# y00njaekim/CMU-11785-IDL-1.58bit-ASR

Hardware: AMD Instinct MI355X
Metric: mel-frames/sec (Conformer-S 1.58-bit train step) (higher is better)
Workload: dtype fp32; 1 GPU; conformer-s-1.58bit-train-step; global_batch=32, execution=hip-graph, per_gpu_batch=32, frames=1000, d_model=144, blocks=16, d_ff=576, heads=4, vocab=5004, parallelism=dp1, passes=teacher 2-bit + student 1-bit + SP, conv_pointwise=fp32 (reference)

## Files before the change

cmu-11785-idl-1.58bit-asr_amd/csrc/capi.hip:

```cpp
#include <float.h>

#include <algorithm>
#include <vector>

#include "../../include/onebit_hip.h"
#include "ob_launch.h"
#include <stdint.h>

using namespace ob;

namespace {

constexpr int kAbiVersion = 4;

inline hipStream_t as_stream(void* s) { return reinterpret_cast<hipStream_t>(s); }

inline bool aligned4(const void* p) { return (reinterpret_cast<uintptr_t>(p) & 3) == 0; }
inline bool misaligned8(const void* p) { return (reinterpret_cast<uintptr_t>(p) & 7) != 0; }

inline int check_bits(int bits) { return (bits == 1 || bits == 2) ? OB_OK : OB_ERR_BITWIDTH; }

inline int launched() {
  const hipError_t e = hipGetLastError();
  return e == hipSuccess ? OB_OK : OB_ERR_HIP;
// ... 2059 lines not shown
  if ((dgamma || dbeta) && ws_bytes < layernorm_bwd_workspace(rows, d)) return OB_ERR_WORKSPACE;
  if (!aligned4(dy) || !aligned4(x) || !aligned4(dx) || !aligned4(dres) || !aligned4(dy2) ||
      !aligned4(lens))
    return OB_ERR_ALIGN;
  if (dy2) {
    if (!(p_drop >= 0.0f && p_drop < 1.0f)) return OB_ERR_SHAPE;
    if (lens && (T < 1 || T > 0x7fffffff || rows % T)) return OB_ERR_SHAPE;
    if (p_drop > 0.0f && !rng) return OB_ERR_NULL;
  }
  LnGradScale gs{dy2, rscale, p_drop, rng, (uint64_t)rng_offset,
                 reinterpret_cast<const int*>(lens), (int)T};
  const LnDefer df{static_cast<LnParamEntry*>(table), (int)slot};
  launch_layernorm_bwd(dy, x, gamma, mean, rstd, rows, d, dres, dx, dgamma, dbeta, ws,
                       as_stream(stream), &gs, &df);
  return launched();
}

namespace {
int relattn_check(int64_t Bt, int64_t P, int64_t T, int64_t H, int64_t d, float p_drop) {
  if (Bt < 1 || P < 1 || Bt % P != 0 || H < 1 || !relattn_supported(T, d)) return OB_ERR_SHAPE;
  if (Bt > 65535 || H > 65535 || !(p_drop >= 0.0f && p_drop < 1.0f)) return OB_ERR_SHAPE;
  return OB_OK;
}
}

int ob_relattn_fwd(const float* q, const float* k, const float* v, const float* pos,
                   const float* u, const float* vb, const int32_t* lens, int64_t Bt, int64_t P,
                   int64_t T, int64_t H, int64_t d, float p_drop, const int64_t* rng,
                   int64_t rng_offset, float* saved, float* probs, float* ctx, void* stream) {
  if (int st = relattn_check(Bt, P, T, H, d, p_drop)) return st;
  if (!q || !k || !v || !pos || !u || !vb || !lens || !ctx || (p_drop > 0.0f && !rng))
    return OB_ERR_NULL;
  if (((uintptr_t)saved & 15) || ((uintptr_t)probs & 15)) return OB_ERR_ALIGN;
  launch_relattn_fwd(q, k, v, pos, u, vb, lens, Bt, P, T, H, d, p_drop,
                     reinterpret_cast<const uint64_t*>(rng), (uint64_t)rng_offset, saved, probs,
                     ctx, as_stream(stream));
  return launched();
}

int64_t ob_relattn_saved_elems(int64_t Bt, int64_t T, int64_t H, int64_t d) {
  if (Bt < 1 || H < 1 || !relattn_supported(T, d)) return 0;
  return relattn_saved_elems(Bt, T, H, d);
}

size_t ob_relattn_bwd_workspace(int64_t Bt, int64_t T, int64_t H, int64_t d) {
  if (Bt < 1 || H < 1 || !relattn_supported(T, d)) return 0;
  return align_up(relattn_bwd_workspace(Bt, T, H, d));
}

int ob_relattn_set_bwd_mode(int mode) { return relattn_set_flash(mode); }

int ob_tgemm_set_colloop(int on) { return tgemm_set_colloop(on); }

int64_t ob_relattn_probs_elems(int64_t Bt, int64_t T, int64_t H) {
  if (Bt < 1 || H < 1 || T < 1) return 0;
  return relattn_probs_elems(Bt, T, H);
}

int ob_relattn_bwd(const float* dctx, const float* ctx, const float* q, const float* k,
                   const float* v, const float* pos, const float* u, const float* vb,
                   const int32_t* lens, int64_t Bt, int64_t P, int64_t T, int64_t H, int64_t d,
                   float p_drop, const int64_t* rng, int64_t rng_offset, const float* saved,
                   int64_t saved_elems, float* dq, float* dk, float* dv, float* dpos, float* du,
                   float* dvb, void* ws, size_t ws_bytes, void* stream) {
  if (int st = relattn_check(Bt, P, T, H, d, p_drop)) return st;
  if (!dctx || !ctx || !q || !k || !v || !pos || !u || !vb || !lens || !saved || !dq || !dk ||
      !dv || !dpos || !du || !dvb || !ws)
    return OB_ERR_NULL;
  if (saved_elems != relattn_saved_elems(Bt, T, H, d)) return OB_ERR_SHAPE;
  (void)rng;
  (void)rng_offset;
  if ((uintptr_t)saved & 15) return OB_ERR_ALIGN;
  if (ws_bytes < ob_relattn_bwd_workspace(Bt, T, H, d)) return OB_ERR_WORKSPACE;
  launch_relattn_bwd(dctx, ctx, q, k, v, pos, u, vb, lens, Bt, P, T, H, d, p_drop, saved, dq, dk,
                     dv, dpos, du, dvb, ws, as_stream(stream));
  return launched();
}

int ob_decattn_supported(int64_t Lq, int64_t Lk, int64_t dh) {
  return decattn_supported(Lq, Lk, dh) ? 1 : 0;
}

static int decattn_check(int64_t B, int64_t H, int64_t Lq, int64_t Lk, int64_t dh, int64_t sq,
                         int64_t sk, int64_t sv, float p_drop) {
  if (B < 0 || H < 1 || !decattn_supported(Lq, Lk, dh) || !(p_drop >= 0.0f && p_drop < 1.0f))
    return OB_ERR_SHAPE;
  if (sq < H * dh || sk < H * dh || sv < H * dh) return OB_ERR_SHAPE;
  if (B * H * Lq > INT32_MAX) return OB_ERR_SHAPE;
  return OB_OK;
}

int ob_decattn_fwd(const float* q, int64_t sq, const float* k, int64_t sk, const float* v,
                   int64_t sv, const uint8_t* kmask, int64_t causal, int64_t B, int64_t H,
                   int64_t Lq, int64_t Lk, int64_t dh, float p_drop, const int64_t* rng,
                   int64_t rng_offset, float* probs, float* ctx, void* stream) {
  if (int st = decattn_check(B, H, Lq, Lk, dh, sq, sk, sv, p_drop)) return st;
  if (B > 0 && (!q || !k || !v || !probs || !ctx || (p_drop > 0.0f && !rng))) return OB_ERR_NULL;
  if (!aligned4(q) || !aligned4(k) || !aligned4(v) || !aligned4(probs) ||
      (reinterpret_cast<uintptr_t>(ctx) & 15))
    return OB_ERR_ALIGN;
  launch_decattn_fwd(q, sq, k, sk, v, sv, kmask, causal ? 1 : 0, B, H, Lq, Lk, dh, p_drop,
                     reinterpret_cast<const uint64_t*>(rng), (uint64_t)rng_offset, probs, ctx,
                     as_stream(stream));
  return launched();
}

// ... 76 lines not shown
```

cmu-11785-idl-1.58bit-asr_amd/csrc/ob_launch.h:

```cpp
#pragma once

#include <hip/hip_runtime.h>
#include <stddef.h>
#include <stdint.h>

#include "../../include/onebit_hip.h"

namespace ob {

inline int64_t ceil_div(int64_t a, int64_t b) { return (a + b - 1) / b; }

void launch_quant_pack(const float* W, const float* alpha, int alpha_raw, int bits,
                       const int* bits_dev, int64_t N, int64_t K, uint32_t* codes,
                       uint32_t* codes_t, hipStream_t s);
int64_t quant_pack_item_blocks(int64_t N, int64_t K);
int64_t quant_pack_item_blocks16(int64_t N, int64_t K);
void launch_quant_pack_group(const ob_pack_item* items_dev, int n_items, int64_t total_blocks,
                             hipStream_t s);
void launch_quant_dequant(const float* W, const float* alpha, int alpha_raw, int bits, int64_t n,
                          float* W_hat, hipStream_t s);

int64_t ste_reduce_blocks(int64_t total);
void launch_ste_reduce(const float* part, int chunks, int64_t nk, const float* part_db,
                       int64_t n_db, const float* W, const float* alpha, int alpha_raw, int bits,
// ... 407 lines not shown
bool ctc_supported(int64_t S);
void launch_ctc_fwd(const float* lp, const int64_t* targets, const int64_t* in_len,
                    const int64_t* tg_len, int64_t B, int64_t T, int64_t V, int64_t S, int blank, int64_t G,
                    float* loss, float* ws, hipStream_t s);
void launch_ctc_bwd(const float* lp, const int64_t* targets, const int64_t* in_len,
                    const int64_t* tg_len, int64_t B, int64_t T, int64_t V, int64_t S, int blank, int64_t G,
                    const float* grad_out, float* grad, float* ws, hipStream_t s);
size_t ctc_logits_workspace_bytes(int64_t B, int64_t T, int64_t S);
void launch_ctc_logits_fwd(const float* x, const int64_t* targets, const int64_t* in_len,
                           const int64_t* tg_len, int64_t B, int64_t T, int64_t V, int64_t S,
                           int blank, int64_t G, float* loss, void* ws, hipStream_t s);
void launch_ctc_logits_bwd(const float* x, const int64_t* targets, const int64_t* in_len,
                           const int64_t* tg_len, int64_t B, int64_t T, int64_t V, int64_t S,
                           int blank, int64_t G, const float* grad_out, float* grad, void* ws,
                           hipStream_t s);

bool att_kl_supported(int64_t V);
size_t att_kl_workspace(int64_t P, int64_t BU);
void launch_att_kl_fwd(const float* x, const int64_t* tgt, const uint8_t* pad, int64_t P,
                       int64_t BU, int64_t V, int pad_id, float ls, float* l_att, float* l_kl,
                       void* ws, hipStream_t s);
void launch_att_kl_bwd(const float* x, const int64_t* tgt, const uint8_t* pad, int64_t P,
                       int64_t BU, int64_t V, float ls, const float* g_att, const float* g_kl,
                       float* grad, const void* ws, hipStream_t s);
void launch_loss_combine_fwd(const float* l_att, const float* l_ctc, const float* l_kl,
                             float gamma, float lam1, float lam2, float* loss, float* parts,
                             hipStream_t s);
void launch_loss_combine_bwd(const float* gl, float gamma, float lam1, float lam2, float* d_att,
                             float* d_ctc, float* d_kl, hipStream_t s);

struct AdamwTensor {
  float* param;
  const float* grad;
  float* exp_avg;
  float* exp_avg_sq;
  int64_t numel;
};
int64_t adamw_plan(const int64_t* numels, int64_t n, int64_t* map);
size_t adamw_workspace(int64_t n_blocks);
void launch_adamw(const AdamwTensor* tab, const int64_t* map, int64_t nb, const float* lr,
                  float* step, float grad_scale, double beta1, double beta2, double eps,
                  double weight_decay, double max_norm, float* total_norm_out, void* ws,
                  hipStream_t s);

bool embed_supported(int64_t C);
void launch_embed_bwd(const int64_t* idx, int64_t N, const float* g, int64_t C, int64_t V,
                      int64_t pad, float* dW, hipStream_t s);

bool relattn_supported(int64_t T, int64_t d);
size_t relattn_bwd_workspace(int64_t Bt, int64_t T, int64_t H, int64_t d);
int64_t relattn_probs_elems(int64_t Bt, int64_t T, int64_t H);
int64_t relattn_saved_elems(int64_t Bt, int64_t T, int64_t H, int64_t d);
int relattn_set_flash(int on);
void launch_relattn_fwd(const float* q, const float* k, const float* v, const float* pos,
                        const float* u, const float* vb, const int* lens, int64_t Bt, int64_t P,
                        int64_t T, int64_t H, int64_t d, float p_drop, const uint64_t* rng,
                        uint64_t rng_off, float* saved, float* probs, float* ctx, hipStream_t s);
void launch_relattn_bwd(const float* dctx, const float* ctx, const float* q, const float* k,
                        const float* v, const float* pos, const float* u, const float* vb,
                        const int* lens, int64_t Bt, int64_t P, int64_t T, int64_t H, int64_t d,
                        float p_drop, const float* saved, float* dq, float* dk, float* dv,
                        float* dpos, float* du, float* dvb, void* ws, hipStream_t s);
void launch_relattn_dropout_mask(int64_t n, int64_t T, float p_drop, const uint64_t* rng,
                                 uint64_t rng_off, uint8_t* out, hipStream_t s);

bool subsample_supported(int64_t T, int64_t F, int64_t C);
size_t subsample_image_bytes(int64_t C);
void launch_subsample_pack(const float* W2, int64_t C, void* img, hipStream_t s);
void launch_subsample_fwd(const float* X, int64_t B, int64_t T, int64_t F, int64_t C,
                          const float* W0, const float* b0, const void* img, const float* b2,
                          float* Y1, float* Y2, hipStream_t s);
size_t subsample_bwd_workspace(int64_t B, int64_t T, int64_t F, int64_t C);
void launch_subsample_bwd(const float* X, const float* W0, const float* b0, const float* Y1,
                          const float* Y2, const float* dY2, int64_t B, int64_t T, int64_t F,
                          int64_t C, const void* img,
                          float* dW0, float* db0, float* dW2, float* db2, void* ws,
                          hipStream_t s);

}
```

cmu-11785-idl-1.58bit-asr_amd/csrc/relattn.hip:

```cpp
#include <atomic>
#include <math.h>

#include <algorithm>

#include "ob_drop.h"
#include "ob_launch.h"
#include "ob_mma.h"

namespace {
template <typename F>
__device__ __forceinline__ uint32_t xrows_1632(uint32_t x, F op) {
  const auto a = __builtin_amdgcn_permlane16_swap(x, x, false, false);
  x = op(a[0], a[1]);
  const auto b = __builtin_amdgcn_permlane32_swap(x, x, false, false);
  return op(b[0], b[1]);
}
__device__ __forceinline__ float xsum_1632(float v) {
  return __builtin_bit_cast(float, xrows_1632(__builtin_bit_cast(uint32_t, v), [](uint32_t a, uint32_t b) {
    return __builtin_bit_cast(uint32_t, __builtin_bit_cast(float, a) + __builtin_bit_cast(float, b));
  }));
}
__device__ __forceinline__ float xmax_1632(float v) {
  return __builtin_bit_cast(float, xrows_1632(__builtin_bit_cast(uint32_t, v), [](uint32_t a, uint32_t b) {
    return __builtin_bit_cast(uint32_t, fmaxf(__builtin_bit_cast(float, a), __builtin_bit_cast(float, b)));
// ... 779 lines not shown
    }
#pragma unroll
    for (int sl = 0; sl < St::kBSlots; ++sl) {
      const int e = threadIdx.x + kThreads * sl;
      if (e >= 2 * St::kBVec) continue;
      const int e2 = e < St::kBVec ? e : e - St::kBVec;
      const int row = e2 / DQ, c4 = 4 * (e2 % DQ);
      if (e < St::kBVec) {
        f32x4 xu, xv;
#pragma unroll
        for (int j = 0; j < 4; ++j) {
          xu[j] = rb[sl][j] + ub[c4 + j];
          xv[j] = rb[sl][j] + vbb[c4 + j];
        }
        *(f32x4*)&st.qu[row][c4] = xu;
        *(f32x4*)&st.qv[row][c4] = xv;
      } else {
        *(f32x4*)&st.dob[row][c4] = rb[sl];
      }
    }
  };

  f32x4 ak[CT], av[CT], ap[CT];
#pragma unroll
  for (int ct = 0; ct < CT; ++ct) {
    ak[ct] = f32x4{0.f, 0.f, 0.f, 0.f};
    av[ct] = f32x4{0.f, 0.f, 0.f, 0.f};
    ap[ct] = f32x4{0.f, 0.f, 0.f, 0.f};
  }
  const int kl = 16 * w + r;
  OB_STAMP_DECL(4)
  fetch(0);
  OB_STAMP(0);
  for (int i0 = 0; i0 < T; i0 += kQ) {
    __syncthreads();
    OB_STAMP(1);
    stage();
    OB_STAMP(2);
    __syncthreads();
    OB_STAMP(3);
    if (i0 + kQ < T) fetch(i0 + kQ);
#pragma unroll
    for (int s4 = 0; s4 < kQ / 4; ++s4) {
      const int qq = 4 * s4 + g;
      const float a_k = st.ak[qq][kl], a_v = st.av[qq][kl], a_p = st.ap[qq][kl];
#pragma unroll
      for (int ct = 0; ct < CT; ++ct) {
        const int col = 16 * ct + r;
        ak[ct] = mfma4(a_k, st.qu[qq][col], ak[ct]);
        av[ct] = mfma4(a_v, st.dob[qq][col], av[ct]);
        ap[ct] = mfma4(a_p, st.qv[qq][col], ap[ct]);
      }
    }
    OB_STAMP(4);
  }
  float* dkb = dk + bo;
  float* dvb = dv + bo;
  float* dpb = dp_part + ((size_t)b * H + h) * T * D;
#pragma unroll
  for (int ct = 0; ct < CT; ++ct) {
    const int col = 16 * ct + r;
    if (col >= D) continue;
#pragma unroll
    for (int j = 0; j < 4; ++j) {
      const int kk = k0 + 16 * w + 4 * g + j;
      if (kk >= T) continue;
      dkb[(size_t)kk * C + col] = ak[ct][j];
      dvb[(size_t)kk * C + col] = av[ct][j];
      dpb[(size_t)kk * D + col] = ap[ct][j];
    }
  }
  OB_STAMP(5);
  OB_STAMP_WRITE(kThreads / 64)
}

constexpr int kFQ = 32;
constexpr int kPlanePitch = 40;

template <int CT>
__device__ __forceinline__ void key_side(const float (&a8)[8], const __bf16* pl, int g, int r,
                                         f32x4 (&acc)[CT]) {
  bf16x8 a[3];
  split3x8(a8, a);
#pragma unroll
  for (int ct = 0; ct < CT; ++ct) {
    bf16x8 bb[3];
#pragma unroll
    for (int pp = 0; pp < 3; ++pp) {
      const __bf16* pu = pl + (size_t)pp * 16 * CT * kPlanePitch + (16 * ct + r) * kPlanePitch + 4 * g;
      const bf16x4 u0 = *(const bf16x4*)pu, u1 = *(const bf16x4*)(pu + 16);
#pragma unroll
      for (int j = 0; j < 4; ++j) {
        bb[pp][j] = u0[j];
        bb[pp][4 + j] = u1[j];
      }
    }
    acc[ct] = mfma_x6(a, bb, acc[ct]);
  }
}

template <int WHICH, int DP>
__device__ __forceinline__ void dq_job(const float* __restrict__ arow, float live,
                                       const float* __restrict__ brow,
                                       __amdgpu_buffer_rsrc_t rs_p, int voff, int C, int sb,
                                       int se, f32x4 (&ac4)[4]) {
#pragma unroll
// ... 528 lines not shown
    if (e >= 2 * n_kv) return;
    const bool isv = e >= n_kv;
    const int64_t i = isv ? e - n_kv : e;
    const float* src = kv_part + (isv ? (int64_t)nqt * n_kv : 0) + i;
    f32x4 acc = *(const f32x4*)src;
    for (int sp = 1; sp < nqt; ++sp) acc += *(const f32x4*)(src + sp * n_kv);
    *(f32x4*)((isv ? dv : dk) + i) = acc;
  }
}

__global__ __launch_bounds__(kThreads) void relattn_mask_kernel(int64_t n, int64_t T, DropCfg dc,
                                                                const uint64_t* __restrict__ rng,
                                                                uint64_t rng_off,
                                                                uint8_t* __restrict__ out) {
  const int64_t e = (int64_t)blockIdx.x * kThreads + threadIdx.x;
  if (e >= n) return;
  const int64_t row = e / T, j = e - row * T;
  const uint64_t idx = (uint64_t)row * (uint64_t)(T + (T & 1)) + (uint64_t)j;
  out[e] = (!dc.on || drop_keep(drop_key(rng[0], rng[1] + rng_off), idx, dc.thresh)) ? 1 : 0;
}

size_t fwd_lds_bytes(int T, int D) {
  const size_t img = sizeof(float) * (size_t)(kTile + 1) * (T + 1);
  const size_t nt = (T + 15) / 16;
  const size_t kp = std::min<size_t>(32 * ((nt + 1) / 2), kFwdKeyChunk);
  const size_t vst = sizeof(uint16_t) * 3 * (size_t)(16 * ((D + 15) / 16)) * (kp + 8);
  return img > vst ? img : vst;
}
size_t bwd_lds_bytes(int T) { return sizeof(float) * ((size_t)(kTile + 1) * T + 128); }

}

bool relattn_supported(int64_t T, int64_t d) {
  return T >= 1 && T <= 512 && (d == 16 || d == 32 || d == 36 || d == 64);
}

static std::atomic<int> g_flash{-1};
static bool flash_selected() {
  int m = g_flash.load(std::memory_order_relaxed);
  if (m < 0) {
    const char* e = getenv("OB_ATTN_BWD");
    int want = (e != nullptr && e[0] == 'f') ? 1 : 0;
    g_flash.compare_exchange_strong(m, want);
    m = g_flash.load(std::memory_order_relaxed);
  }
  return m == 1;
}
int relattn_set_flash(int on) {
  const int prev = flash_selected() ? 1 : 0;
  if (on == 0 || on == 1) g_flash.store(on, std::memory_order_relaxed);
  return prev;
}
bool relattn_fused(int64_t T, int64_t d) { return T <= 256 && d <= 36 && flash_selected(); }

struct SavedLayout {
  int64_t stats, kbits, tail, total;
  SavedLayout(int64_t Bt, int64_t T, int64_t H, int64_t d) {
    const int64_t nt = (T + 15) / 16, Tp = 16 * nt, W = (nt + 1) / 2, nch = (Tp + 31) / 32;
    stats = 0;
    kbits = Bt * H * Tp * 2;
    tail = kbits + Bt * H * Tp * W;
    tail = (tail + 3) & ~(int64_t)3;
    total = tail + (relattn_fused(T, d) ? Bt * H * nch * T : relattn_probs_elems(Bt, T, H));
  }
};

int64_t relattn_saved_elems(int64_t Bt, int64_t T, int64_t H, int64_t d) {
  return SavedLayout(Bt, T, H, d).total;
}

int64_t relattn_probs_elems(int64_t Bt, int64_t T, int64_t H) {
  const int64_t nt = (T + 15) / 16;
  return Bt * H * nt * nt * 256;
}

int fused_splits(int64_t T) { return ((16 * ((T + 15) / 16) + 31) / 32) >= 2 ? 2 : 1; }

size_t relattn_bwd_workspace(int64_t Bt, int64_t T, int64_t H, int64_t d) {
  if (relattn_fused(T, d)) {
    const int64_t ns = fused_splits(T);
    const int64_t kv = ns > 1 ? 2 * ns * Bt * T * H * d + 4 : 0;
    return sizeof(float) * (size_t)(Bt * H * ns * T * d + 2 * Bt * H * ns * d + kv + 64);
  }
  const int64_t nqt = (T + kTile - 1) / kTile;
  return sizeof(float) * (size_t)(Bt * H * T * T + Bt * H * T * d + 2 * Bt * H * nqt * d + 64);
}

#define OB_RA_DISPATCH(KERNEL)                 \
  do {                                         \
    const bool big = T > 256;                  \
    if (d == 16) {                             \
      if (big) KERNEL(4, 32); else KERNEL(4, 16);   \
    } else if (d == 32) {                      \
      if (big) KERNEL(8, 32); else KERNEL(8, 16);   \
    } else if (d == 36) {                      \
      if (big) KERNEL(9, 32); else KERNEL(9, 16);   \
    } else {                                   \
      if (big) KERNEL(16, 32); else KERNEL(16, 16); \
    }                                          \
  } while (0)

void launch_relattn_fwd(const float* q, const float* k, const float* v, const float* pos,
                        const float* u, const float* vb, const int* lens, int64_t Bt, int64_t P,
                        int64_t T, int64_t H, int64_t d, float p_drop, const uint64_t* rng,
                        uint64_t rng_off, float* saved, float* probs, float* ctx, hipStream_t s) {
  const dim3 grid((unsigned)(((T + kTile - 1) / kTile) * H * Bt));
// ... 25 lines not shown
  if (relattn_fused(T, d)) {
    const DropCfg dc = make_drop(p_drop);
    const float inv_sqrt_d = 1.0f / (float)sqrt((double)d);
    const int ns = fused_splits(T);
    const int64_t C = H * d;
    const int64_t n_kv = Bt * T * C;
    float* dp_part = (float*)ws;
    float* du_part = dp_part + (size_t)Bt * H * ns * T * d;
    float* dvb_part = du_part + (size_t)Bt * H * ns * d;
    float* kv_part = dvb_part + (size_t)Bt * H * ns * d;
    kv_part += (16 - ((uintptr_t)kv_part & 15)) / 4 % 4;
    const SavedLayout sl(Bt, T, H, d);
    const float* stats = saved;
    const uint32_t* kbits = reinterpret_cast<const uint32_t*>(saved + sl.kbits);
    const float* anchors = saved + sl.tail;
    const int CT = (int)((d + 15) / 16);
    const size_t lds = sizeof(float) * FusedLds((int)T, (int)d, CT, (int)((Tp + kFQ - 1) / kFQ), (int)W).total;
    float* dk_out = ns > 1 ? kv_part : dk;
    float* dv_out = ns > 1 ? kv_part + ns * n_kv : dv;
#define OB_RA_FUSED(DQ)                                                                           \
  hipLaunchKernelGGL((relattn_bwd_fused_kernel<DQ, kFusedWaves>), dim3((unsigned)(Bt * H * ns)),   \
                     dim3(64 * kFusedWaves), lds, s, dctx, ctx, q, k, v, pos, u, vb, lens, stats,   \
                     kbits, anchors, (int)(Bt / P), (int)T, (int)H, ns, inv_sqrt_d, dc, dq, dk_out, \
                     dv_out, (size_t)n_kv, dp_part, du_part, dvb_part)
    if (d == 16) OB_RA_FUSED(4);
    else if (d == 32) OB_RA_FUSED(8);
    else OB_RA_FUSED(9);
#undef OB_RA_FUSED
    const int n_dpos = (int)ceil_div(P * T * C, 64);
    const int n_bias = (int)(2 * H * ((d + kBiasCols - 1) / kBiasCols));
    const int n_kvb = ns > 1 ? (int)ceil_div(2 * n_kv, 4 * kThreads) : 0;
    hipLaunchKernelGGL(relattn_reduce_kernel, dim3((unsigned)(n_dpos + n_bias + n_kvb)),
                       dim3(kThreads), 0, s, (const float*)dp_part, (const float*)du_part,
                       (const float*)dvb_part, (int)Bt, (int)P, (int)T, (int)H, (int)d, ns, n_dpos,
                       dpos, du, dvb, ns, n_bias, (const float*)kv_part, n_kv, dk, dv);
    return;
  }
  const float* probs = saved + SavedLayout(Bt, T, H, d).tail;
  const int nqt = (int)((T + kTile - 1) / kTile);
  const dim3 grid((unsigned)(nqt * H * Bt));
  const DropCfg dc = make_drop(p_drop);
  const float inv_sqrt_d = 1.0f / (float)sqrt((double)d);
  const size_t lds = bwd_lds_bytes((int)T);
  float* dsg = (float*)ws;
  float* dp_part = dsg + (size_t)Bt * H * T * T;
  float* du_part = dp_part + (size_t)Bt * H * T * d;
  float* dvb_part = du_part + (size_t)Bt * H * nqt * d;
#define OB_RA_BWD(DQ, NTT)                                                                     \
  hipLaunchKernelGGL((relattn_bwd_kernel<DQ, NTT>), grid, dim3(kThreads), lds, s, dctx, ctx, k,    \
                     v, pos, (int)(Bt / P), (int)T, (int)H, inv_sqrt_d, dc, probs, dq, dsg,        \
                     du_part, dvb_part)
  OB_RA_DISPATCH(OB_RA_BWD);
#undef OB_RA_BWD
#define OB_RA_KV(DQ, NTT)                                                                          \
  hipLaunchKernelGGL((relattn_bwd_kv_kernel<DQ>), grid, dim3(kThreads), 0, s, (const float*)dsg,    \
                     probs, q, dctx, u, vb, (int)T, (int)H, dc, dk, dv, dp_part)
  OB_RA_DISPATCH(OB_RA_KV);
#undef OB_RA_KV
  const int64_t C = H * d;
  const int n_dpos = (int)ceil_div(P * T * C, 64);
  const int n_bias = (int)(2 * H * ((d + kBiasCols - 1) / kBiasCols));
  hipLaunchKernelGGL(relattn_reduce_kernel, dim3((unsigned)(n_dpos + n_bias)), dim3(kThreads), 0, s,
                     (const float*)dp_part, (const float*)du_part, (const float*)dvb_part, (int)Bt,
                     (int)P, (int)T, (int)H, (int)d, nqt, n_dpos, dpos, du, dvb, 1, n_bias,
                     (const float*)nullptr, (int64_t)0, (float*)nullptr, (float*)nullptr);
}

#ifdef OB_ATTN_STAMPS
extern "C" int ob_attn_stamps(void* host_dst) {
  return hipMemcpyFromSymbol(host_dst, HIP_SYMBOL(g_attn_stamps), sizeof(g_attn_stamps)) == hipSuccess ? 0 : -6;
}
extern "C" int ob_attn_rt(void* host_dst) {
  return hipMemcpyFromSymbol(host_dst, HIP_SYMBOL(g_attn_rt), sizeof(g_attn_rt)) == hipSuccess ? 0 : -6;
}
#endif

void launch_relattn_dropout_mask(int64_t n, int64_t T, float p_drop, const uint64_t* rng,
                                 uint64_t rng_off, uint8_t* out, hipStream_t s) {
  if (n == 0) return;
  hipLaunchKernelGGL(relattn_mask_kernel, dim3((unsigned)((n + kThreads - 1) / kThreads)),
                     dim3(kThreads), 0, s, n, T, make_drop(p_drop), rng, rng_off, out);
}

}
```

cmu-11785-idl-1.58bit-asr_amd/onebit_asr/_lib.py:

```python
from __future__ import annotations

import ctypes
import os
from pathlib import Path

import torch

LIB_NAME = "libonebit_hip.so"
LIB_PATH = Path(os.environ.get("ONEBIT_HIP_LIB") or Path(__file__).with_name(LIB_NAME))

OB_OK = 0
OB_ERR_SHAPE = -2
OB_ERR_BITWIDTH = -3

_c_f = ctypes.c_void_p
_i64 = ctypes.c_int64
_int = ctypes.c_int
_sz = ctypes.c_size_t
_f32 = ctypes.c_float
_f64 = ctypes.c_double

SIGNATURES = {
    "ob_abi_version": (_int, []),
    "ob_source_digest": (ctypes.c_char_p, []),
# ... 201 lines not shown
               _sz, _c_f, _i64, _i64, _c_f, _c_f]),
    "ob_bitlinear_bwd_dw_passes_group_defer": (
        _int, [_i64, _c_f, _c_f, _i64, _i64, _i64, _i64, _c_f, _c_f, _int, _c_f, _c_f, _c_f, _c_f,
               _c_f, _sz, _c_f, _i64, _i64, _c_f, _c_f]),
    "ob_dw_finish_table": (_int, [_c_f, _i64, _i64, _c_f]),
    "ob_dw_grouped_supported": (_int, [_i64, _i64]),
    "ob_dw_grouped_workspace": (_sz, [_c_f, _i64]),
    "ob_dw_grouped_tickets": (_sz, [_c_f, _i64]),
    "ob_dw_grouped": (_int, [_c_f, _i64, _c_f, _sz, _c_f, _sz, _c_f]),
    "ob_dense_dw_defer": (_int, [_c_f, _c_f, _i64, _i64, _i64, _c_f, _c_f, _c_f, _sz, _c_f, _i64,
                                 _i64, _c_f, _c_f]),
    "ob_layernorm_bwd_workspace": (_sz, [_i64, _i64]),
    "ob_layernorm_bwd": (
        _int, [_c_f, _c_f, _c_f, _c_f, _c_f, _i64, _i64, _c_f, _c_f, _c_f, _c_f, _sz, _c_f]),
    "ob_layernorm_bwd_res": (
        _int, [_c_f, _c_f, _c_f, _c_f, _c_f, _i64, _i64, _c_f, _c_f, _c_f, _c_f, _c_f, _sz, _c_f]),
    "ob_layernorm_bwd_ex": (
        _int, [_c_f, _c_f, _c_f, _c_f, _c_f, _i64, _i64, _c_f, _c_f, _c_f, _c_f, _c_f, _sz, _c_f,
               _f32, _f32, _c_f, _i64, _c_f, _i64, _c_f]),
    "ob_act_absmax_workspace": (_sz, [_i64]),
    "ob_act_absmax": (_int, [_c_f, _i64, _i64, _c_f, _c_f, _sz, _c_f]),
    "ob_act_dequant_i8": (_int, [_c_f, _i64, _i64, _c_f, _c_f, _c_f]),
    "ob_bitlinear_fwd_i8": (
        _int, [_c_f, _i64, _i64, _i64, _c_f, _c_f, _c_f, _c_f, _int, _c_f, _c_f, _i64, _c_f, _c_f]),
    "ob_bitlinear_fwd_i8_epi": (
        _int, [_c_f, _i64, _i64, _i64, _c_f, _c_f, _c_f, _c_f, _int, _c_f, _c_f, _i64, _int, _c_f,
               _f32, _c_f, _i64, _c_f, _c_f, _c_f]),
    "ob_bitlinear_fwd_passes_group": (
        _int, [_i64, _c_f, _i64, _i64, _i64, _c_f, _c_f, _c_f, _c_f, _int, _c_f, _i64, _c_f, _c_f]),
    "ob_bitlinear_fwd_i8q": (
        _int, [_c_f, _i64, _i64, _i64, _c_f, _c_f, _c_f, _c_f, _int, _c_f, _c_f, _i64, _int, _c_f,
               _f32, _c_f, _i64, _c_f, _c_f, _c_f]),
    "ob_bitlinear_bwd_dx_passes": (
        _int, [_c_f, _i64, _i64, _i64, _c_f, _c_f, _c_f, _c_f, _int, _i64, _c_f, _c_f]),
    "ob_bitlinear_bwd_dw_passes_workspace": (_sz, [_i64, _i64, _i64, _i64]),
    "ob_bitlinear_bwd_dw_passes": (
        _int, [_c_f, _c_f, _i64, _i64, _i64, _i64, _c_f, _c_f, _int, _c_f, _c_f, _c_f, _c_f, _c_f,
               _sz, _c_f]),
    "ob_bitlinear_bwd_dw_passes_group_workspace": (_sz, [_i64, _i64, _i64, _i64, _i64]),
    "ob_bitlinear_bwd_dw_passes_group": (
        _int, [_i64, _c_f, _c_f, _i64, _i64, _i64, _i64, _c_f, _c_f, _int, _c_f, _c_f, _c_f, _c_f,
               _c_f, _sz, _c_f]),
    "ob_relattn_fwd": (
        _int, [_c_f, _c_f, _c_f, _c_f, _c_f, _c_f, _c_f, _i64, _i64, _i64, _i64, _i64, _f32, _c_f,
               _i64, _c_f, _c_f, _c_f, _c_f]),
    "ob_relattn_saved_elems": (_i64, [_i64, _i64, _i64, _i64]),
    "ob_relattn_probs_elems": (_i64, [_i64, _i64, _i64]),
    "ob_relattn_bwd_workspace": (_sz, [_i64, _i64, _i64, _i64]),
    "ob_relattn_bwd": (
        _int, [_c_f, _c_f, _c_f, _c_f, _c_f, _c_f, _c_f, _c_f, _c_f, _i64, _i64, _i64, _i64, _i64,
               _f32, _c_f, _i64, _c_f, _i64, _c_f, _c_f, _c_f, _c_f, _c_f, _c_f, _c_f, _sz, _c_f]),
    "ob_relattn_set_bwd_mode": (_int, [_int]),
    "ob_tgemm_set_colloop": (_int, [_int]),
    "ob_relattn_dropout_mask": (_int, [_i64, _i64, _f32, _c_f, _i64, _c_f, _c_f]),
    "ob_embedding_bwd": (_int, [_c_f, _i64, _c_f, _i64, _i64, _i64, _c_f, _c_f]),
    "ob_adamw_plan": (_i64, [_c_f, _i64, _c_f]),
    "ob_adamw_workspace": (_sz, [_i64]),
    "ob_adamw_clip_step": (
        _int, [_c_f, _i64, _c_f, _i64, _c_f, _c_f, _f32, _f64, _f64, _f64, _f64, _f64, _c_f, _c_f,
               _sz, _c_f]),
}

ABI_VERSION = 4

_lib = None


class OneBitHipError(RuntimeError):
    pass


def load() -> ctypes.CDLL:
    global _lib
    if _lib is not None:
        return _lib
    if not LIB_PATH.is_file():
        raise OneBitHipError(
            f"{LIB_PATH} is missing: build it with `make -C cmu-11785-idl-1.58bit-asr_amd/csrc` "
            "(or __graft_entry__.build()); there is no CPU fallback for the BitLinear path"
        )
    lib = ctypes.CDLL(str(LIB_PATH))
    for name, (res, args) in SIGNATURES.items():
        fn = getattr(lib, name)
        fn.restype = res
        fn.argtypes = args
    if lib.ob_abi_version() != ABI_VERSION:
        raise OneBitHipError(f"ABI mismatch: library {lib.ob_abi_version()} != {ABI_VERSION}")
    check_digest(lib)
    _lib = lib
    return lib


def check_digest(lib, expected: str | None = None) -> None:
    if expected is None:
        if os.environ.get("ONEBIT_HIP_LIB"):
            return
        if not _sources_present():
            import warnings

            warnings.warn(f"{LIB_PATH.name}: no csrc/ sources beside it; build digest not checked")
            return
        expected = source_digest()
    got = lib.ob_source_digest().decode()
    if got != expected:
        raise OneBitHipError(
            f"{LIB_PATH.name} was built from other sources (digest {got[:12]} != {expected[:12]} "
# ... 34 lines not shown
```

include/onebit_hip.h:

```cpp
#ifndef ONEBIT_HIP_H_
#define ONEBIT_HIP_H_

#include <stddef.h>
#include <stdint.h>

#ifdef __cplusplus
extern "C" {
#endif

#define OB_API __attribute__((visibility("default")))

enum {
  OB_OK = 0,
  OB_ERR_NULL = -1,
  OB_ERR_SHAPE = -2,
  OB_ERR_BITWIDTH = -3,
  OB_ERR_WORKSPACE = -4,
  OB_ERR_ALIGN = -5,
  OB_ERR_HIP = -6
};

OB_API int ob_abi_version(void);
OB_API const char* ob_source_digest(void);
OB_API const char* ob_status_string(int status);
// ... 181 lines not shown
    void* ws, size_t ws_bytes, void* table, int64_t slot, int64_t start, int64_t* n_blocks,
    void* stream);
OB_API int ob_dw_finish_table(const void* table, int64_t n, int64_t total_blocks, void* stream);

typedef struct ob_dwg_gemm {
  const float* dY;
  const float* X;
  const float* W;
  const float* alpha;
  const int32_t* pass_bits;
  float* dW;
  float* db;
  float* dalpha;
  int64_t N, K, M, P;
  int32_t alpha_raw, bits;
} ob_dwg_gemm;
OB_API int ob_dw_grouped_supported(int64_t N, int64_t K);
OB_API size_t ob_dw_grouped_workspace(const ob_dwg_gemm* gemms, int64_t G);
OB_API size_t ob_dw_grouped_tickets(const ob_dwg_gemm* gemms, int64_t G);
OB_API int ob_dw_grouped(const ob_dwg_gemm* gemms, int64_t G, void* ws, size_t ws_bytes,
                         void* tickets, size_t ticket_words, void* stream);

OB_API int ob_decattn_supported(int64_t Lq, int64_t Lk, int64_t dh);
OB_API int ob_decattn_fwd(const float* q, int64_t sq, const float* k, int64_t sk, const float* v,
                          int64_t sv, const uint8_t* kmask, int64_t causal, int64_t B, int64_t H,
                          int64_t Lq, int64_t Lk, int64_t dh, float p_drop, const int64_t* rng,
                          int64_t rng_offset, float* probs, float* ctx, void* stream);
OB_API int ob_decattn_bwd(const float* dctx, const float* ctx, const float* q, int64_t sq,
                          const float* k, int64_t sk, const float* v, int64_t sv, int64_t B, int64_t H, int64_t Lq,
                          int64_t Lk, int64_t dh, float p_drop, float* probs, float* dq,
                          int64_t gq, float* dk, int64_t gk, float* dv, int64_t gv, void* stream);
OB_API int ob_decattn_fwd_grouped(const float* q, int64_t sq, const float* k, int64_t sk,
                                  const float* v, int64_t sv, const uint8_t* kmask,
                                  int64_t causal, int64_t B, int64_t kv_group, int64_t H,
                                  int64_t Lq, int64_t Lk, int64_t dh, float* ctx, void* stream);

OB_API int ob_relattn_fwd(const float* q, const float* k, const float* v, const float* pos,
                          const float* u, const float* vb, const int32_t* lens, int64_t Bt,
                          int64_t P, int64_t T, int64_t H, int64_t d, float p_drop,
                          const int64_t* rng, int64_t rng_offset, float* saved, float* probs,
                          float* ctx, void* stream);
OB_API int64_t ob_relattn_saved_elems(int64_t Bt, int64_t T, int64_t H, int64_t d);
OB_API int64_t ob_relattn_probs_elems(int64_t Bt, int64_t T, int64_t H);
OB_API size_t ob_relattn_bwd_workspace(int64_t Bt, int64_t T, int64_t H, int64_t d);
OB_API int ob_relattn_bwd(const float* dctx, const float* ctx, const float* q, const float* k,
                          const float* v, const float* pos, const float* u, const float* vb,
                          const int32_t* lens, int64_t Bt, int64_t P, int64_t T, int64_t H,
                          int64_t d, float p_drop, const int64_t* rng, int64_t rng_offset,
                          const float* saved, int64_t saved_elems,
                          float* dq, float* dk, float* dv, float* dpos, float* du, float* dvb,
                          void* ws, size_t ws_bytes, void* stream);
OB_API int ob_relattn_set_bwd_mode(int mode);
OB_API int ob_tgemm_set_colloop(int on);
OB_API int ob_relattn_dropout_mask(int64_t n, int64_t row_len, float p_drop, const int64_t* rng,
                                   int64_t rng_offset, uint8_t* out, void* stream);

OB_API int ob_embedding_bwd(const int64_t* indices, int64_t N, const float* grad, int64_t C,
                            int64_t V, int64_t padding_idx, float* grad_weight, void* stream);

typedef struct ob_adamw_tensor {
  float* param;
  const float* grad;
  float* exp_avg;
  float* exp_avg_sq;
  int64_t numel;
} ob_adamw_tensor;

OB_API int64_t ob_adamw_plan(const int64_t* numels, int64_t n_tensors, int64_t* chunk_map);
OB_API size_t ob_adamw_workspace(int64_t n_blocks);
OB_API int ob_adamw_clip_step(const ob_adamw_tensor* table, int64_t n_tensors,
                              const int64_t* chunk_map, int64_t n_blocks, const float* lr,
                              float* step, float grad_scale, double beta1, double beta2,
                              double eps, double weight_decay, double max_norm,
                              float* total_norm, void* ws,
                              size_t ws_bytes, void* stream);

OB_API int ob_layernorm_fwd(const float* x, const float* gamma, const float* beta, int64_t rows,
                            int64_t d, float eps, float* y, float* mean, float* rstd,
                            void* stream);
OB_API int ob_layernorm_fwd_pair(const float* x, const float* g1, const float* b1,
                                 const float* g2, const float* b2, int64_t rows, int64_t d,
                                 float eps1, float eps2, float* y1, float* mean1, float* rstd1,
                                 float* y2, float* mean2, float* rstd2, void* stream);
OB_API size_t ob_layernorm_fwd_amax_workspace(int64_t P);
OB_API int ob_layernorm_fwd_amax(const float* x, const float* gamma, const float* beta,
                                 int64_t rows, int64_t d, float eps, float* y, float* mean,
                                 float* rstd, int64_t P, float* amax, void* ws,
                                 size_t ws_bytes, void* stream);
OB_API int ob_layernorm_fwd_i8(const float* x, const float* gamma, const float* beta,
                               int64_t rows, int64_t d, float eps, int64_t P, float* amax,
                               int8_t* yq, void* ws, size_t ws_bytes, void* stream);
OB_API size_t ob_layernorm_bwd_workspace(int64_t rows, int64_t d);
OB_API int ob_layernorm_bwd(const float* dy, const float* x, const float* gamma,
                            const float* mean, const float* rstd, int64_t rows, int64_t d,
                            float* dx, float* dgamma, float* dbeta, void* ws, size_t ws_bytes,
                            void* stream);
OB_API int ob_layernorm_bwd_res(const float* dy, const float* x, const float* gamma,
                                const float* mean, const float* rstd, int64_t rows, int64_t d,
                                const float* dres, float* dx, float* dgamma, float* dbeta,
                                void* ws, size_t ws_bytes, void* stream);
OB_API int ob_layernorm_bwd_ex(const float* dy, const float* x, const float* gamma,
                               const float* mean, const float* rstd, int64_t rows, int64_t d,
                               const float* dres, float* dx, float* dgamma, float* dbeta,
                               void* ws, size_t ws_bytes, float* dy2, float rscale,
                               float p_drop, const uint64_t* rng, int64_t rng_offset,
                               const int32_t* lens, int64_t T, void* stream);
// ... 275 lines not shown
```

Baseline: 1.416 million mel-frames/s.

## Add double-buffered LDS ring variant of relative-attention dK/dV backward kernel

Adds a new dK/dV/dpos backward kernel that splits the shared-memory stage into two 16-query buffers used as a ping-pong ring. While one buffer feeds the MFMA accumulation, the next chunk's global loads and LDS writes proceed, which is meant to hide load latency behind compute at the same LDS footprint and occupancy. A runtime switch, on by default, selects the ring kernel over the original one. The cost is an extra barrier per 16 queries and more code to maintain.

Result: faster. 1.436 million mel-frames/s (median of 6 runs) (+1.4%).

```diff
diff --git a/cmu-11785-idl-1.58bit-asr_amd/csrc/capi.hip b/cmu-11785-idl-1.58bit-asr_amd/csrc/capi.hip
--- a/cmu-11785-idl-1.58bit-asr_amd/csrc/capi.hip
+++ b/cmu-11785-idl-1.58bit-asr_amd/csrc/capi.hip
@@ -2135,6 +2135,8 @@
 
 int ob_tgemm_set_colloop(int on) { return tgemm_set_colloop(on); }
 
+int ob_relattn_set_kv_ring(int on) { return relattn_set_kv_ring(on); }
+
 int64_t ob_relattn_probs_elems(int64_t Bt, int64_t T, int64_t H) {
   if (Bt < 1 || H < 1 || T < 1) return 0;
   return relattn_probs_elems(Bt, T, H);
diff --git a/cmu-11785-idl-1.58bit-asr_amd/csrc/ob_launch.h b/cmu-11785-idl-1.58bit-asr_amd/csrc/ob_launch.h
--- a/cmu-11785-idl-1.58bit-asr_amd/csrc/ob_launch.h
+++ b/cmu-11785-idl-1.58bit-asr_amd/csrc/ob_launch.h
@@ -483,6 +483,7 @@
 int64_t relattn_probs_elems(int64_t Bt, int64_t T, int64_t H);
 int64_t relattn_saved_elems(int64_t Bt, int64_t T, int64_t H, int64_t d);
 int relattn_set_flash(int on);
+int relattn_set_kv_ring(int on);
 void launch_relattn_fwd(const float* q, const float* k, const float* v, const float* pos,
                         const float* u, const float* vb, const int* lens, int64_t Bt, int64_t P,
                         int64_t T, int64_t H, int64_t d, float p_drop, const uint64_t* rng,
diff --git a/cmu-11785-idl-1.58bit-asr_amd/csrc/relattn.hip b/cmu-11785-idl-1.58bit-asr_amd/csrc/relattn.hip
--- a/cmu-11785-idl-1.58bit-asr_amd/csrc/relattn.hip
+++ b/cmu-11785-idl-1.58bit-asr_amd/csrc/relattn.hip
@@ -855,6 +855,212 @@
         ap[ct] = mfma4(a_p, st.qv[qq][col], ap[ct]);
       }
     }
+    OB_STAMP(4);
+  }
+  float* dkb = dk + bo;
+  float* dvb = dv + bo;
+  float* dpb = dp_part + ((size_t)b * H + h) * T * D;
+#pragma unroll
+  for (int ct = 0; ct < CT; ++ct) {
+    const int col = 16 * ct + r;
+    if (col >= D) continue;
+#pragma unroll
+    for (int j = 0; j < 4; ++j) {
+      const int kk = k0 + 16 * w + 4 * g + j;
+      if (kk >= T) continue;
+      dkb[(size_t)kk * C + col] = ak[ct][j];
+      dvb[(size_t)kk * C + col] = av[ct][j];
+      dpb[(size_t)kk * D + col] = ap[ct][j];
+    }
+  }
+  OB_STAMP(5);
+  OB_STAMP_WRITE(kThreads / 64)
+}
+
+template <int D>
+struct KvRing {
+  static constexpr int kQ = 16;
+  static constexpr int kAP = KvStage<D>::kAP;
+  static constexpr int kBP = KvStage<D>::kBP;
+  static constexpr int kBVec = kQ * (D / 4);
+  static constexpr int kBSlots = (kBVec + kThreads - 1) / kThreads;
+  struct Stage {
+    alignas(16) float ak[kQ][kAP];
+    alignas(16) float av[kQ][kAP];
+    alignas(16) float ap[kQ][kAP];
+    alignas(16) float qu[kQ][kBP];
+    alignas(16) float qv[kQ][kBP];
+    alignas(16) float dob[kQ][kBP];
+  };
+  Stage s[2];
+};
+static_assert(sizeof(KvRing<36>) == sizeof(KvStage<36>) && sizeof(KvRing<64>) == sizeof(KvStage<64>),
+              "the ring keeps the 32-query chunk's LDS footprint (three blocks per CU at d = 36)");
+
+template <int DQ>
+__global__ __launch_bounds__(kThreads) void relattn_bwd_kv_ring_kernel(
+    const float* __restrict__ dsg, const float* __restrict__ probs, const float* __restrict__ q,
+    const float* __restrict__ dctx, const float* __restrict__ u, const float* __restrict__ vbias,
+    int T, int H, DropCfg dc, float* __restrict__ dk, float* __restrict__ dv,
+    float* __restrict__ dp_part) {
+  constexpr int D = 4 * DQ;
+  constexpr int CT = (D + 15) / 16;
+  using Rg = KvRing<D>;
+  using Stage = typename Rg::Stage;
+  constexpr int kQ = Rg::kQ;
+  __shared__ Rg rg;
+  const int nt = (T + 15) >> 4;
+  const int nkt = (T + kTile - 1) / kTile;
+  const BlockId bid = block_id(nkt, H);
+  const int b = bid.b, h = bid.h, k0 = bid.qt * kTile;
+  const int bh = b * H + h;
+  const int C = H * D;
+  const int lane = threadIdx.x & 63, w = threadIdx.x >> 6, r = lane & 15, g = lane >> 4;
+  const size_t bo = (size_t)b * T * C + h * D;
+  const float* qb = q + bo;
+  const float* dob = dctx + bo;
+  const float* ub = u + h * D;
+  const float* vbb = vbias + h * D;
+  const float* dsb = dsg + (size_t)bh * T * T;
+  const float* prb = probs + frag_off(bh, 0, 0, nt);
+
+  constexpr int kPad = Rg::kBP - D;
+  for (int e = threadIdx.x; e < 2 * kQ * kPad; e += kThreads) {
+    Stage& S = rg.s[e / (kQ * kPad)];
+    const int row = (e / kPad) % kQ, c = D + e % kPad;
+    S.qu[row][c] = 0.0f;
+    S.qv[row][c] = 0.0f;
+    S.dob[row][c] = 0.0f;
+  }
+
+  const int ai = threadIdx.x >> 4, ax = 4 * (threadIdx.x & 15);
+  const int key0 = k0 + ax;
+  const size_t pcol = (size_t)256 * (key0 >> 4) + 64 * ((key0 & 15) >> 2);
+  const int eq0 = threadIdx.x, eo0 = kThreads - 1 - (int)threadIdx.x;
+  f32x4 ra_k, ra_v, ra_p, rq[Rg::kBSlots], ro[Rg::kBSlots];
+  const __amdgpu_buffer_rsrc_t rs_ds = __builtin_amdgcn_make_buffer_rsrc(
+      const_cast<float*>(dsb), (short)0, (int)((size_t)T * T * sizeof(float)), 0x00020000);
+  const __amdgpu_buffer_rsrc_t rs_pr = __builtin_amdgcn_make_buffer_rsrc(
+      const_cast<float*>(prb), (short)0, (int)((size_t)nt * nt * 256 * sizeof(float)), 0x00020000);
+  const __amdgpu_buffer_rsrc_t rs_q = slice_rsrc(qb, T, C, D), rs_do = slice_rsrc(dob, T, C, D);
+  const bool kfull = key0 + 3 < T;
+  f32x4 ubr[Rg::kBSlots], vbr[Rg::kBSlots];
+#pragma unroll
+  for (int sl = 0; sl < Rg::kBSlots; ++sl) {
+    const int e = eq0 + kThreads * sl;
+    const int c4 = 4 * (e % DQ);
+#pragma unroll
+    for (int j = 0; j < 4; ++j) {
+      ubr[sl][j] = e < Rg::kBVec ? ub[c4 + j] : 0.0f;
+      vbr[sl][j] = e < Rg::kBVec ? vbb[c4 + j] : 0.0f;
+    }
+  }
+  auto a_whole = [&](int i) { return kfull && i < T && i * (T + 1) + key0 + 1 - T >= 0; };
+  auto fetch = [&](int i0) {
+    const int i = i0 + ai;
+    const int fk = i * T + key0, fx = i * (T + 1) + key0 + 1 - T;
+    if (a_whole(i)) {
+      ra_k = __builtin_amdgcn_raw_buffer_load_b128(rs_ds, 4 * fk, 0, 0);
+      ra_p = __builtin_amdgcn_raw_buffer_load_b128(rs_ds, 4 * fx, 0, 0);
+    } else {
+#pragma unroll
+      for (int j = 0; j < 4; ++j) {
+        ra_k[j] = __builtin_bit_cast(float, __builtin_amdgcn_raw_buffer_load_b32(rs_ds, 4 * (fk + j), 0, 0));
+        ra_p[j] = __builtin_bit_cast(float, __builtin_amdgcn_raw_buffer_load_b32(rs_ds, 4 * max(fx + j, 0), 0, 0));
+      }
+    }
+    ra_v = key0 < 16 * nt
+               ? __builtin_amdgcn_raw_buffer_load_b128(
+                     rs_pr, 4 * (int)((size_t)(i >> 4) * nt * 256 + pcol + 4 * (i & 15)), 0, 0)
+               : f32x4{0.f, 0.f, 0.f, 0.f};
+#pragma unroll
+    for (int sl = 0; sl < Rg::kBSlots; ++sl) {
+      const int eq = eq0 + kThreads * sl, eo = eo0 + kThreads * sl;
+      if (eq < Rg::kBVec)
+        rq[sl] = __builtin_amdgcn_raw_buffer_load_b128(rs_q, 4 * ((i0 + eq / DQ) * C + 4 * (eq % DQ)), 0, 0);
+      if (eo < Rg::kBVec)
+        ro[sl] = __builtin_amdgcn_raw_buffer_load_b128(rs_do, 4 * ((i0 + eo / DQ) * C + 4 * (eo % DQ)), 0, 0);
+    }
+  };
+  auto write = [&](Stage& S, int i0) {
+    const int i = i0 + ai;
+    if (!a_whole(i)) {
+      const int fx = i * (T + 1) + key0 + 1 - T;
+#pragma unroll
+      for (int j = 0; j < 4; ++j) {
+        const bool ok = i < T && key0 + j < T;
+        ra_k[j] = ok ? ra_k[j] : 0.0f;
+        ra_p[j] = ok && fx + j >= 0 ? ra_p[j] : 0.0f;
+      }
+    }
+#pragma unroll
+    for (int j = 0; j < 4; ++j) {
+      if (dc.on) ra_v[j] = __builtin_signbit(ra_v[j]) ? 0.0f : ra_v[j] * dc.scale;
+    }
+    *(f32x4*)&S.ak[ai][ax] = ra_k;
+    *(f32x4*)&S.av[ai][ax] = ra_v;
+    *(f32x4*)&S.ap[ai][ax] = ra_p;
+#pragma unroll
+    for (int sl = 0; sl < Rg::kBSlots; ++sl) {
+      const int eq = eq0 + kThreads * sl, eo = eo0 + kThreads * sl;
+      if (eq < Rg::kBVec) {
+        f32x4 xu, xv;
+#pragma unroll
+        for (int j = 0; j < 4; ++j) {
+          xu[j] = rq[sl][j] + ubr[sl][j];
+          xv[j] = rq[sl][j] + vbr[sl][j];
+        }
+        *(f32x4*)&S.qu[eq / DQ][4 * (eq % DQ)] = xu;
+        *(f32x4*)&S.qv[eq / DQ][4 * (eq % DQ)] = xv;
+      }
+      if (eo < Rg::kBVec) *(f32x4*)&S.dob[eo / DQ][4 * (eo % DQ)] = ro[sl];
+    }
+  };
+
+  f32x4 ak[CT], av[CT], ap[CT];
+#pragma unroll
+  for (int ct = 0; ct < CT; ++ct) {
+    ak[ct] = f32x4{0.f, 0.f, 0.f, 0.f};
+    av[ct] = f32x4{0.f, 0.f, 0.f, 0.f};
+    ap[ct] = f32x4{0.f, 0.f, 0.f, 0.f};
+  }
+  const int kl = 16 * w + r;
+  auto mma = [&](const Stage& S) {
+#pragma unroll
+    for (int s4 = 0; s4 < kQ / 4; ++s4) {
+      const int qq = 4 * s4 + g;
+      const float a_k = S.ak[qq][kl], a_v = S.av[qq][kl], a_p = S.ap[qq][kl];
+#pragma unroll
+      for (int ct = 0; ct < CT; ++ct) {
+        const int col = 16 * ct + r;
+        ak[ct] = mfma4(a_k, S.qu[qq][col], ak[ct]);
+        av[ct] = mfma4(a_v, S.dob[qq][col], av[ct]);
+        ap[ct] = mfma4(a_p, S.qv[qq][col], ap[ct]);
+      }
+    }
+  };
+  OB_STAMP_DECL(4)
+  fetch(0);
+  write(rg.s[0], 0);
+  fetch(kQ);
+  OB_STAMP(0);
+  for (int i0 = 0; i0 < T; i0 += 2 * kQ) {
+    const bool more = i0 + 2 * kQ < T;
+    __syncthreads();
+    OB_STAMP(1);
+    write(rg.s[1], i0 + kQ);
+    if (more) fetch(i0 + 2 * kQ);
+    OB_STAMP(2);
+    mma(rg.s[0]);
+    OB_STAMP(4);
+    __syncthreads();
+    OB_STAMP(1);
+    if (more) {
+      write(rg.s[0], i0 + 2 * kQ);
+      fetch(i0 + 3 * kQ);
+    }
+    OB_STAMP(2);
+    mma(rg.s[1]);
     OB_STAMP(4);
   }
   float* dkb = dk + bo;
@@ -1489,6 +1695,13 @@
   return prev;
 }
 bool relattn_fused(int64_t T, int64_t d) { return T <= 256 && d <= 36 && flash_selected(); }
+
+static std::atomic<int> g_kv_ring{1};
+int relattn_set_kv_ring(int on) {
+  const int prev = g_kv_ring.load(std::memory_order_relaxed);
+  if (on == 0 || on == 1) g_kv_ring.store(on, std::memory_order_relaxed);
+  return prev;
+}
 
 struct SavedLayout {
   int64_t stats, kbits, tail, total;
@@ -1620,9 +1833,18 @@
                      du_part, dvb_part)
   OB_RA_DISPATCH(OB_RA_BWD);
 #undef OB_RA_BWD
+  const bool ring = g_kv_ring.load(std::memory_order_relaxed) == 1;
 #define OB_RA_KV(DQ, NTT)                                                                          \
-  hipLaunchKernelGGL((relattn_bwd_kv_kernel<DQ>), grid, dim3(kThreads), 0, s, (const float*)dsg,    \
-                     probs, q, dctx, u, vb, (int)T, (int)H, dc, dk, dv, dp_part)
+  do {                                                                                             \
+    if (ring)                                                                                      \
+      hipLaunchKernelGGL((relattn_bwd_kv_ring_kernel<DQ>), grid, dim3(kThreads), 0, s,              \
+                         (const float*)dsg, probs, q, dctx, u, vb, (int)T, (int)H, dc, dk, dv,      \
+                         dp_part);                                                                 \
+    else                                                                                           \
+      hipLaunchKernelGGL((relattn_bwd_kv_kernel<DQ>), grid, dim3(kThreads), 0, s,                   \
+                         (const float*)dsg, probs, q, dctx, u, vb, (int)T, (int)H, dc, dk, dv,      \
+                         dp_part);                                                                 \
+  } while (0)
   OB_RA_DISPATCH(OB_RA_KV);
 #undef OB_RA_KV
   const int64_t C = H * d;
diff --git a/cmu-11785-idl-1.58bit-asr_amd/onebit_asr/_lib.py b/cmu-11785-idl-1.58bit-asr_amd/onebit_asr/_lib.py
--- a/cmu-11785-idl-1.58bit-asr_amd/onebit_asr/_lib.py
+++ b/cmu-11785-idl-1.58bit-asr_amd/onebit_asr/_lib.py
@@ -277,6 +277,7 @@
                _f32, _c_f, _i64, _c_f, _i64, _c_f, _c_f, _c_f, _c_f, _c_f, _c_f, _c_f, _sz, _c_f]),
     "ob_relattn_set_bwd_mode": (_int, [_int]),
     "ob_tgemm_set_colloop": (_int, [_int]),
+    "ob_relattn_set_kv_ring": (_int, [_int]),
     "ob_relattn_dropout_mask": (_int, [_i64, _i64, _f32, _c_f, _i64, _c_f, _c_f]),
     "ob_embedding_bwd": (_int, [_c_f, _i64, _c_f, _i64, _i64, _i64, _c_f, _c_f]),
     "ob_adamw_plan": (_i64, [_c_f, _i64, _c_f]),
diff --git a/include/onebit_hip.h b/include/onebit_hip.h
--- a/include/onebit_hip.h
+++ b/include/onebit_hip.h
@@ -257,6 +257,7 @@
                           void* ws, size_t ws_bytes, void* stream);
 OB_API int ob_relattn_set_bwd_mode(int mode);
 OB_API int ob_tgemm_set_colloop(int on);
+OB_API int ob_relattn_set_kv_ring(int on);
 OB_API int ob_relattn_dropout_mask(int64_t n, int64_t row_len, float p_drop, const int64_t* rng,
                                    int64_t rng_offset, uint8_t* out, void* stream);
 
```
